# Shinokawa/Fast-SCNN-pytorch

Measured on AMD Instinct MI355X. Metric: images/sec fwd+bwd @1024x2048 bs=8 per GPU; 1/2/4/8-GPU scaling, higher is better.
Workload: dtype bf16; 1 GPU; cfg3 train step: fwd + CE(ignore -1) + bwd + fused SGD (fused low-res upsample+CE head); model=FastSCNN (19 classes), global_batch=8, per_gpu_batch=8, parallelism=dp1

## Files before the change

fast-scnn-pytorch_amd/_lib.py:

```python
import ctypes
import os
import threading

_HERE = os.path.dirname(os.path.abspath(__file__))
LIB_PATH = os.environ.get("FSCNN_LIB", os.path.join(_HERE, "libfastscnn_hip.so"))

DT_F32, DT_BF16, DT_F16 = 0, 1, 2
DT_U8 = 3

c_int, c_ll, c_float, c_vp, c_char_p = (ctypes.c_int, ctypes.c_longlong, ctypes.c_float,
                                        ctypes.c_void_p, ctypes.c_char_p)
c_ull, c_double = ctypes.c_ulonglong, ctypes.c_double
P_int, P_ll, P_vp = ctypes.POINTER(c_int), ctypes.POINTER(c_ll), ctypes.POINTER(c_vp)
P_float = ctypes.POINTER(c_float)
P_double = ctypes.POINTER(c_double)

SIGNATURES = {
    "fscnn_version": (c_char_p, []),
    "fscnn_last_error": (c_char_p, []),
    "fscnn_net_create": (c_int, [c_int, c_int, P_vp]),
    "fscnn_net_destroy": (None, [c_vp]),
    "fscnn_net_param_count": (c_int, [c_vp, P_int, P_ll]),
    "fscnn_net_param_info": (c_int, [c_vp, c_int, ctypes.POINTER(c_char_p), P_ll, P_ll]),
    "fscnn_net_buffer_count": (c_int, [c_vp, P_int, P_ll, P_int]),
# ... 58 lines not shown
    "fscnn_dice_head_ws_bytes": (c_ll, [c_vp]),
    "fscnn_forward_loss_dice": (c_int, [c_vp, c_vp, c_int, c_vp, c_float, c_float, c_float,
                                        c_float, c_float, c_vp, c_vp, c_vp, c_vp, c_vp, c_vp, c_vp,
                                        c_ull, c_float, c_float, c_vp]),
    "fscnn_backward_loss_dice": (c_int, [c_vp, c_vp, c_vp, c_float, c_float, c_float, c_vp, c_int,
                                         c_vp, c_vp, c_vp, c_vp, c_vp, c_ull, c_float, c_int,
                                         c_int, c_vp]),
    "fscnn_forward_loss_ohem": (c_int, [c_vp, c_vp, c_int, c_vp, c_ll, c_float, c_ll, c_vp, c_vp,
                                        c_vp, c_vp, c_vp, c_vp, c_vp, c_vp, c_vp, c_vp, c_ull,
                                        c_float, c_float, c_vp]),
    "fscnn_backward_dx": (c_int, [c_vp, c_vp, c_vp, c_vp, c_vp, c_vp, c_int, c_vp, c_int, c_vp,
                                  c_vp, c_vp, c_vp, c_ull, c_float, c_int, c_int, c_vp]),
    "fscnn_prof_begin": (c_int, [c_int, c_int]),
    "fscnn_prof_end": (c_int, [ctypes.POINTER(ctypes.c_double), P_ll, ctypes.POINTER(ctypes.c_double),
                               ctypes.POINTER(ctypes.c_double)]),
    "fscnn_prof_launch": (c_int, [c_ll, ctypes.POINTER(c_int), ctypes.POINTER(ctypes.c_float),
                                  ctypes.POINTER(ctypes.c_double), ctypes.POINTER(ctypes.c_double),
                                  ctypes.POINTER(c_char_p)]),
    "fscnn_prof_kind_name": (c_char_p, [c_int]),
    "fscnn_ce_parts": (c_ll, [c_int, c_ll]),
    "fscnn_ce_fwd": (c_int, [c_vp, c_int, c_vp, c_int, c_int, c_ll, c_ll, c_vp, c_vp, c_vp]),
    "fscnn_ce_bwd": (c_int, [c_vp, c_int, c_vp, c_int, c_int, c_ll, c_ll, c_vp, c_vp, c_vp,
                             c_vp]),
    "fscnn_sgd": (c_int, [c_vp, c_vp, c_vp, c_ll, c_float, c_float, c_float, c_float, c_int,
                          c_int, c_float, c_vp]),
    "fscnn_adamw": (c_int, [c_vp, c_vp, c_vp, c_vp, c_vp, c_ll, c_double, c_double, c_double,
                            c_double, c_double, c_int, c_int, c_vp, c_int, c_vp, c_vp, c_vp]),
    "fscnn_adamw_segments": (c_int, [c_vp, c_vp, c_vp, c_vp, c_vp, c_vp, c_vp, c_int, c_vp, c_int,
                                     c_vp, c_int, c_vp, c_int, c_int, c_vp, c_vp, c_vp]),
    "fscnn_conv0_fwd": (c_int, [c_vp, c_int, c_int, c_int, c_int, c_vp, c_vp, c_vp, c_int, c_vp,
                                c_int, c_vp]),
    "fscnn_conv0_wgrad_slab_floats": (c_ll, [c_int, c_int, c_int]),
    "fscnn_conv0_wgrad": (c_int, [c_vp, c_int, c_int, c_int, c_int, c_vp, c_int, c_vp, c_vp, c_vp]),
    "fscnn_dw3x3_fwd": (c_int, [c_vp, c_int, c_int, c_int, c_int, c_int, c_int, c_vp, c_vp, c_vp,
                                c_int, c_vp, c_vp]),
    "fscnn_dw3x3_dgrad": (c_int, [c_vp, c_int, c_int, c_int, c_int, c_int, c_int, c_vp, c_vp,
                                  c_vp]),
    "fscnn_dw3x3_wgrad_slab_floats": (c_ll, [c_int, c_int, c_int, c_int, c_int, c_int]),
    "fscnn_dw3x3_wgrad": (c_int, [c_vp, c_vp, c_int, c_int, c_int, c_int, c_int, c_int, c_vp,
                                  c_vp, c_vp]),
    "fscnn_pw_gemm": (c_int, [c_int, c_int, c_int, c_vp, c_int, c_vp, c_int, c_int, c_vp, c_vp,
                              c_vp, c_int, c_int, c_vp, c_int, c_vp, c_int, c_vp]),
    "fscnn_pw_dgrad_bnbwd": (c_int, [c_int, c_int, c_int, c_vp, c_int, c_vp, c_int, c_vp, c_int,
                                     c_vp, c_int, c_vp, c_int, c_vp, c_vp, c_vp, c_vp, c_int,
                                     c_vp, c_vp, c_vp, c_vp, c_vp, c_vp, c_int, P_int, c_vp]),
    "fscnn_kth_smallest": (c_int, [c_vp, c_ll, c_ll, c_vp, c_vp, c_vp]),
    "fscnn_debug_stamps": (c_int, [c_vp, c_int]),
    "fscnn_debug_stamp_count": (c_int, []),
    "fscnn_debug_stamp_tag": (c_char_p, [c_int]),
    "fscnn_pw_wgrad_slab_floats": (c_ll, [c_int, c_int, c_int]),
    "fscnn_pw_gemm_stats_parts": (c_int, [c_int, c_int, c_int, c_int, c_int, c_int]),
    "fscnn_pw_wgrad": (c_int, [c_int, c_int, c_int, c_vp, c_int, c_vp, c_int, c_vp, c_vp, c_int,
                               c_vp]),
    "fscnn_bn_finalize": (c_int, [c_vp, c_int, c_int, c_vp, c_vp, c_vp, c_vp, c_vp, c_float,
                                  c_vp, c_vp, c_vp, c_vp, c_vp]),
    "fscnn_bilinear_ac_fwd": (c_int, [c_vp, c_int, c_int, c_int, c_int, c_int, c_int, c_int,
                                      c_vp, c_int, c_int, c_vp]),
    "fscnn_bilinear_ac_bwd": (c_int, [c_vp, c_int, c_int, c_int, c_int, c_int, c_int, c_int,
                                      c_vp, c_vp, c_vp]),
    "fscnn_pyramid_pool_fwd": (c_int, [c_vp, c_int, c_int, c_int, c_int, c_int, c_int, c_vp,
                                       c_vp]),
    "fscnn_block_ir_fwd": (c_int, [c_vp, c_int, c_int, c_int, c_int, c_int, c_int, c_int, c_int,
                                   c_vp, c_vp, c_vp, c_vp, c_vp, c_vp, c_vp, c_vp, c_vp, c_int,
                                   c_vp, c_int, c_vp]),
    "fscnn_pyramid_pool_bwd": (c_int, [c_vp, c_int, c_int, c_int, c_int, c_int, c_vp, c_int,
                                       c_int, c_vp]),
    "fscnn_block_ir_s2_fwd": (c_int, [c_vp, c_int, c_int, c_int, c_int, c_int, c_int, c_int, c_int,
                                      c_vp, c_vp, c_vp, c_vp, c_vp, c_vp, c_vp, c_vp, c_vp, c_vp,
                                      c_int, c_vp]),
    "fscnn_block_ltd_fwd": (c_int, [c_vp, c_int, c_int, c_int, c_int, c_int, c_vp, c_vp, c_vp,
                                    c_vp, c_vp, c_vp, c_vp, c_vp, c_vp, c_vp, c_int, c_vp]),
    "fscnn_block_dsconv_fwd": (c_int, [c_vp, c_int, c_int, c_int, c_int, c_int, c_int, c_vp, c_vp,
                                       c_vp, c_vp, c_vp, c_vp, c_vp, c_int, c_vp]),
    "fscnn_block_dsconv_res_fwd": (c_int, [c_vp, c_int, c_int, c_int, c_int, c_int, c_int, c_int,
                                           c_int, c_vp, c_vp, c_vp, c_vp, c_vp, c_vp, c_vp, c_int,
                                           c_vp, c_int, c_vp]),
    "fscnn_block_cls_fwd": (c_int, [c_vp, c_int, c_int, c_int, c_int] + [c_vp] * 14 + [c_int, c_vp, c_vp,
                                                                              c_int, c_vp]),
    "fscnn_block_ffm_fwd": (c_int, [c_vp, c_int, c_int, c_int, c_int, c_int, c_int, c_vp, c_int,
                                    c_vp, c_vp, c_vp, c_vp, c_vp, c_vp, c_vp, c_vp, c_vp, c_vp,
                                    c_int, c_vp]),
}

_lib = None
_lock = threading.Lock()


def load():
    global _lib
    if _lib is not None:
        return _lib
    with _lock:
        if _lib is not None:
            return _lib
        if not os.path.exists(LIB_PATH):
            raise RuntimeError(
                "libfastscnn_hip.so not found at %s — build it with "
                "`python -c 'import __graft_entry__; __graft_entry__.build()'` "
                "(there is no CPU fallback)" % LIB_PATH)
        import torch
        lib = ctypes.CDLL(LIB_PATH, mode=ctypes.RTLD_GLOBAL)
        for name, (res, args) in SIGNATURES.items():
            fn = getattr(lib, name)
            fn.restype = res
            fn.argtypes = args
        _lib = lib
# ... 34 lines not shown
```

fast-scnn-pytorch_amd/csrc/capi.cpp:

```cpp
#include <algorithm>
#include <chrono>
#include <cmath>
#include <cstdlib>
#include <cstdarg>
#include <cstdio>
#include <cstring>
#include <new>
#include <string>

#include "../../include/fastscnn.h"
#include "net.hpp"

namespace fscnn {

static thread_local char g_err[512] = "";

void set_error(const char* fmt, ...) {
  va_list ap;
  va_start(ap, fmt);
  vsnprintf(g_err, sizeof g_err, fmt, ap);
  va_end(ap);
}
const char* last_error() { return g_err; }

// ... 961 lines not shown

int fscnn_pw_gemm_stats_parts(int M, int N, int K, int lda, int ldc, int dtype) {
  GemmArgs a{};
  static float dummy;
  a.M = M; a.N = N; a.K = K; a.lda = lda; a.ldb = K; a.ldc = ldc; a.part = &dummy;
  return gemm_nt_parts(a, dtype);
}
int fscnn_pw_gemm(int M, int N, int K, const void* A, int lda, const void* B, int ldb,
                  int b_trans, const float* scale, const float* shift, const void* R, int ldr,
                  int relu, void* C, int ldc, float* stats_part, int dtype, void* stream) {
  GemmArgs a{};
  a.M = M; a.N = N; a.K = K; a.A = A; a.lda = lda; a.B = B; a.ldb = ldb; a.b_trans = b_trans;
  a.scale = scale; a.shift = shift; a.R = R; a.ldr = ldr; a.relu = relu; a.C = C; a.ldc = ldc;
  a.part = stats_part;
  return gemm_nt(a, dtype, S(stream));
}
int fscnn_pw_dgrad_bnbwd(int M, int N, int K, const void* D, int ldd, const void* B, int ldb,
                         const void* R, int ldr, void* dX, int lddx, const void* z, int ldz,
                         const float* mean, const float* invstd, const float* scale,
                         const float* shift, int relu_mode, float* part, unsigned* counters,
                         double* tsum, float* dgamma, float* dbeta, float* coef, int dtype,
                         int* path, void* stream) {
  if (!D || !B || !dX || !z || !mean || !invstd || !scale || !shift || !part || !counters ||
      !tsum || !dgamma || !dbeta || !coef) {
    set_error("fscnn_pw_dgrad_bnbwd: null argument");
    return E_INVALID;
  }
  if (dtype < DT_F32 || dtype > DT_F16 || (relu_mode != 0 && relu_mode != 2)) {
    set_error("fscnn_pw_dgrad_bnbwd: dtype %d / relu_mode %d", dtype, relu_mode);
    return E_INVALID;
  }
  GemmArgs a{};
  a.M = M; a.N = N; a.K = K; a.A = D; a.lda = ldd; a.B = B; a.ldb = ldb; a.b_trans = 0;
  a.R = R; a.ldr = ldr; a.C = dX; a.ldc = lddx;
  a.bpart = part; a.bz = z; a.ldbz = ldz;
  a.bmean = mean; a.binvstd = invstd; a.bscale = scale; a.bshift = shift; a.bmode = relu_mode;
  a.tail.counters = counters; a.tail.tsum = tsum; a.tail.count = (double)M;
  a.tail.dgamma = dgamma; a.tail.dbeta = dbeta; a.tail.coef = coef;
  if (path) *path = gemm_stream_ok(a, dtype) ? 1 : 0;
  return gemm_nt(a, dtype, S(stream));
}
long long fscnn_pw_wgrad_slab_floats(int M, int N, int K) {
  return (long long)gemm_tn_splits(M, N, K) * N * K;
}
int fscnn_pw_wgrad(int M, int N, int K, const void* D, int ldd, const void* X, int ldx,
                   float* slab, float* dW, int dtype, void* stream) {
  GemmTnArgs a{};
  a.M = M; a.N = N; a.K = K; a.D = D; a.ldd = ldd; a.X = X; a.ldx = ldx; a.slab = slab;
  int s = gemm_tn_splits(M, N, K);
  int rc = gemm_tn(a, s, dtype, S(stream));
  if (rc) return rc;
  return reduce_slabs(slab, s, (long long)N * K, (long long)N * K, dW, 0, S(stream));
}

int fscnn_bn_finalize(float* part, int P, int C, const float* gamma, const float* beta,
                      float* rmean, float* rvar, long long* nbt, float momentum, float* mean,
                      float* invstd, float* scale, float* shift, void* stream) {
  BnFinalizeArgs a{};
  a.part = part; a.P = P; a.C = C; a.gamma = gamma; a.beta = beta; a.rmean = rmean;
  a.rvar = rvar; a.nbt = nbt; a.momentum = momentum; a.mean = mean; a.invstd = invstd;
  a.scale = scale; a.shift = shift;
  return bn_finalize(a, S(stream));
}

int fscnn_bilinear_ac_fwd(const void* x, int dtype, int N, int Hi, int Wi, int C, int Ho, int Wo,
                          void* y, int out_nchw, int out_dtype, void* stream) {
  UpArgs a{};
  a.N = N; a.Hi = Hi; a.Wi = Wi; a.C = C; a.Ho = Ho; a.Wo = Wo; a.x = x; a.ldx = C; a.y = y;
  a.ldy = C;
  if (out_nchw) return up_nchw(a, dtype, out_dtype, S(stream));
  return up_nhwc(a, dtype, S(stream));
}
int fscnn_bilinear_ac_bwd(const void* dy, int dtype, int N, int Hi, int Wi, int C, int Ho, int Wo,
                          float* tmp, void* dx, void* stream) {
  AxisBwdArgs a{};
  a.n_o1 = (long long)N * Ho; a.n_o2 = 1; a.Lout = Wo; a.Lin = Wi; a.n_in = C;
  a.g = dy; a.g_s1 = (long long)Wo * C; a.g_idx = C; a.g_in = 1;
  a.d = tmp; a.d_s1 = (long long)Wi * C; a.d_idx = C; a.d_in = 1;
  int rc = axis_bwd(a, dtype, DT_F32, S(stream));
  if (rc) return rc;
  AxisBwdArgs b{};
  b.n_o1 = N; b.n_o2 = 1; b.Lout = Ho; b.Lin = Hi; b.n_in = (long long)Wi * C;
  b.g = tmp; b.g_s1 = (long long)Ho * Wi * C; b.g_idx = (long long)Wi * C; b.g_in = 1;
  b.d = dx; b.d_s1 = (long long)Hi * Wi * C; b.d_idx = (long long)Wi * C; b.d_in = 1;
  return axis_bwd(b, DT_F32, dtype, S(stream));
}
int fscnn_pyramid_pool_fwd(const void* x, int dtype, int N, int H, int W, int C, int ldx,
                           void* pooled, void* stream) {
  PoolArgs a{};
  a.N = N; a.H = H; a.W = W; a.C = C; a.x = x; a.ldx = ldx; a.pooled = pooled;
  return pyramid_pool(a, dtype, S(stream));
}
int fscnn_pyramid_pool_bwd(const void* dpooled, int dtype, int N, int H, int W, int C, void* dx,
                           int lddx, int accumulate, void* stream) {
  PoolBwdArgs a{};
  a.N = N; a.H = H; a.W = W; a.C = C; a.dpooled = dpooled; a.dx = dx; a.lddx = lddx;
  a.accumulate = accumulate;
  return pyramid_pool_bwd(a, dtype, S(stream));
}

int fscnn_block_ir_fwd(const void* x, int ldx, int dtype, int N, int H, int W, int cin, int expand,
                       int cout, const void* w_expand, const float* w_dw, const void* w_project,
                       const float* scale_e, const float* shift_e, const float* scale_d,
                       const float* shift_d, const float* scale_p, const float* shift_p,
                       int residual, void* y, int ldy, void* stream) {
  if (!x || !y || !w_expand || !w_dw || !w_project || !scale_e || !shift_e || !scale_d ||
// ... 190 lines not shown
```

fast-scnn-pytorch_amd/csrc/gemm.hip:

```cpp
#include "bn_finish.hpp"

namespace fscnn {


constexpr int G_BM = 128;
constexpr int G_VROW = 8;
constexpr int G_VPAD = 9;
constexpr int G_ATMAX = 768;

template <typename T>
struct MfmaOp;

template <>
struct MfmaOp<float> {
  static __device__ __forceinline__ void run(const uint4& a, const uint4& b, f32x4& acc) {
    acc = __builtin_amdgcn_mfma_f32_16x16x4f32(__uint_as_float(a.x), __uint_as_float(b.x), acc, 0, 0, 0);
    acc = __builtin_amdgcn_mfma_f32_16x16x4f32(__uint_as_float(a.y), __uint_as_float(b.y), acc, 0, 0, 0);
    acc = __builtin_amdgcn_mfma_f32_16x16x4f32(__uint_as_float(a.z), __uint_as_float(b.z), acc, 0, 0, 0);
    acc = __builtin_amdgcn_mfma_f32_16x16x4f32(__uint_as_float(a.w), __uint_as_float(b.w), acc, 0, 0, 0);
  }
};

template <>
struct MfmaOp<bf16> {
  static __device__ __forceinline__ void run(const uint4& a, const uint4& b, f32x4& acc) {
    i16x8 av, bv;
    __builtin_memcpy(&av, &a, 16);
    __builtin_memcpy(&bv, &b, 16);
    acc = __builtin_amdgcn_mfma_f32_16x16x32_bf16(av, bv, acc, 0, 0, 0);
  }
};

template <>
struct MfmaOp<f16> {
  static __device__ __forceinline__ void run(const uint4& a, const uint4& b, f32x4& acc) {
    h16x8 av, bv;
    __builtin_memcpy(&av, &a, 16);
    __builtin_memcpy(&bv, &b, 16);
    acc = __builtin_amdgcn_mfma_f32_16x16x32_f16(av, bv, acc, 0, 0, 0);
  }
};

template <typename T>
__device__ __forceinline__ uint4 zero_tail(uint4 v, int valid) {
  constexpr int V = VecW<T>::V;
  uint32_t w[4] = {v.x, v.y, v.z, v.w};
  if (V == 4) {
#pragma unroll
    for (int j = 0; j < 4; ++j) w[j] = j < valid ? w[j] : 0u;
  } else {
#pragma unroll
    for (int j = 0; j < 4; ++j) {
// ... 650 lines not shown
  };
  using Pair = typename std::conditional<sizeof(T) == 2, uint32_t, uint2>::type;
  if (mb < me) load(mb);
  for (int mc = mb; mc < me; mc += TN_MC) {
    mask(mc);
    __syncthreads();
#pragma unroll
    for (int i = 0; i < PAIRS; ++i) {
      const int id = tid + 256 * i;
      const int rp = id / VPR, vv = id - rp * VPR;
      const T* d0 = reinterpret_cast<const T*>(&rd[i][0]);
      const T* d1 = reinterpret_cast<const T*>(&rd[i][1]);
      const T* x0 = reinterpret_cast<const T*>(&rx[i][0]);
      const T* x1 = reinterpret_cast<const T*>(&rx[i][1]);
#pragma unroll
      for (int j = 0; j < V; ++j) {
        const int n = vv * V + j;
        const int off = n * LD + swz(n, 2 * rp);
        Pair pd, px;
        __builtin_memcpy(reinterpret_cast<T*>(&pd), d0 + j, sizeof(T));
        __builtin_memcpy(reinterpret_cast<T*>(&pd) + 1, d1 + j, sizeof(T));
        __builtin_memcpy(reinterpret_cast<T*>(&px), x0 + j, sizeof(T));
        __builtin_memcpy(reinterpret_cast<T*>(&px) + 1, x1 + j, sizeof(T));
        *reinterpret_cast<Pair*>(&sDt[off]) = pd;
        *reinterpret_cast<Pair*>(&sXt[off]) = px;
      }
    }
    __syncthreads();
    if (mc + TN_MC < me) load(mc + TN_MC);
#pragma unroll
    for (int ks = 0; ks < TN_MC / 32; ++ks) {
      const int kb = ks * 32 + 8 * lq;
#pragma unroll
      for (int i = 0; i < 2; ++i)
#pragma unroll
        for (int j = 0; j < 2; ++j) {
          const int na = wn + i * 16 + li, nb = wk + j * 16 + li;
          TnOps<T>::mma(&sDt[na * LD + swz(na, kb)], &sXt[nb * LD + swz(nb, kb)], acc[i][j]);
        }
    }
  }
  float* sl = a.slab + (size_t)split * a.N * a.K;
#pragma unroll
  for (int i = 0; i < 2; ++i)
#pragma unroll
    for (int j = 0; j < 2; ++j)
#pragma unroll
      for (int r = 0; r < 4; ++r) {
        int n = n0 + wn + i * 16 + lq * 4 + r, k = k0 + wk + j * 16 + li;
        if (n < a.N && k < a.K) sl[(size_t)n * a.K + k] = acc[i][j][r];
      }
}

int gemm_tn_splits(int M, int N, int K) {
  constexpr int target = 512;
  int tiles = cdiv(N, TN_T) * cdiv(K, TN_T);
  int s = target / tiles;
  int smax = cdiv(M, 4 * TN_MC);
  if (s > smax) s = smax;
  if (s >= 8) s &= ~7;
  if (s < 1) s = 1;
  return s;
}

int gemm_tn(GemmTnArgs a, int splits, int dtype, hipStream_t st) {
  const int V = dtype == DT_F32 ? 4 : 8;
  if (a.ldd % V || a.ldx % V || (uintptr_t)a.D % 16 || (uintptr_t)a.X % 16) {
    set_error("gemm_tn: operands must be 16-B aligned (ldd=%d ldx=%d)", a.ldd, a.ldx);
    return E_INVALID;
  }
  a.rows_per_split = cdiv(cdiv(a.M, splits), TN_MC) * TN_MC;
  a.splits = splits;
  dim3 grid(cdiv(a.N, TN_T) * cdiv(a.K, TN_T) * splits);
  const double E = dtype == DT_F32 ? 4.0 : 2.0;
  const double M = a.M, N = a.N, K = a.K;
  ProfScope ps(PK_GEMM_TN, st, E * (M * N + M * K) + 4.0 * N * K, 2.0 * M * N * K);
  const bool xt = a.x_scale != nullptr;
  if (xt && (!a.x_shift || a.K % V)) {
    set_error("gemm_tn: lazy BN on X needs x_shift and K %% %d == 0", V);
    return E_UNSUPPORTED;
  }
#define TN_LAUNCH(T)                                        \
  do {                                                      \
    if (xt) prof_launch(gemm_tn_kernel<T, true>, grid, 256, 0, st, a); \
    else prof_launch(gemm_tn_kernel<T, false>, grid, 256, 0, st, a);   \
  } while (0)
  if (dtype == DT_F32) TN_LAUNCH(float);
  else if (dtype == DT_F16) TN_LAUNCH(f16);
  else TN_LAUNCH(bf16);
#undef TN_LAUNCH
  return check_launch("gemm_tn");
}

constexpr int RED_Q = 64;

__global__ void reduce_fold_kernel(float* slab, int S, int Q, long long stride, int count) {
  int i = blockIdx.x * blockDim.x + threadIdx.x;
  int q = blockIdx.y;
  if (i >= count) return;
  float s = 0.f;
  for (int k0 = q; k0 < S; k0 += 8 * Q) {
    float v[8];
#pragma unroll
    for (int u = 0; u < 8; ++u) {
      const int k = k0 + u * Q;
      const float t = slab[(size_t)(k < S ? k : q) * stride + i];
      v[u] = k < S ? t : 0.f;
    }
#pragma unroll
    for (int u = 0; u < 8; ++u) s += v[u];
  }
  slab[(size_t)q * stride + i] = s;
}

__global__ void reduce_final_kernel(const float* slab, int S, long long stride, int count,
                                    float* out, int accumulate, int C9) {
  int i = blockIdx.x * blockDim.x + threadIdx.x;
  if (i >= count) return;
  float s = 0.f;
  for (int k0 = 0; k0 < S; k0 += 8) {
    float v[8];
#pragma unroll
    for (int u = 0; u < 8; ++u) {
      const float t = slab[(size_t)(k0 + u < S ? k0 + u : 0) * stride + i];
      v[u] = k0 + u < S ? t : 0.f;
    }
#pragma unroll
    for (int u = 0; u < 8; ++u) s += v[u];
  }
  int o = C9 ? (i % C9) * 9 + i / C9 : i;
  out[o] = accumulate ? out[o] + s : s;
}

int reduce_slabs_ex(float* slab, int S, long long stride, long long count, float* out,
                    int accumulate, int C9, hipStream_t st) {
  if (count <= 0 || count > 0x7fffffff) { set_error("reduce_slabs: bad count"); return E_INVALID; }
  int n = (int)count;
  int S2 = S;
  if (S > RED_Q) {
    dim3 g1(cdiv(n, 256), RED_Q);
    prof_launch(reduce_fold_kernel, g1, 256, 0, st, slab, S, RED_Q, stride, n);
    S2 = RED_Q;
// ... 125 lines not shown
```

fast-scnn-pytorch_amd/csrc/kernels.hpp:

```cpp
#pragma once
#include "common.hpp"

namespace fscnn {

constexpr int MAX_FOLD = 48;
constexpr double BN_FROZEN_COUNT = -1.0;


struct Conv0Args {
  const void* x;
  int x_bf16;
  int N, H, W, Ho, Wo;
  const float* w;
  const float* scale;
  const float* shift;
  int relu;
  void* y;
  float* part;
  unsigned long long* stamps = nullptr;
};

struct Conv0WgradArgs {
  const void* x;
  int x_bf16;
// ... 459 lines not shown
  unsigned long long* stamps = nullptr;
};
bool ds2_ok(const Ds2Args& a);
int ds2_fwd(const Ds2Args& a, int dtype, hipStream_t st);
int ds_rows(int N, int H, int W);
int ds_fwd(const DsArgs& a, int dtype, hipStream_t st);

struct Conv0DgradArgs {
  const void* dz;
  const float* w;
  int N, H, W, Ho, Wo;
  void* dx;
  int dx_dtype;
};
int conv0_dgrad(const Conv0DgradArgs& a, int dz_dtype, hipStream_t st);
int conv0_parts(int N, int Ho, int Wo);
int conv0_fwd(const Conv0Args& a, int y_dtype, hipStream_t st);
int conv0_wgrad_parts(int N, int Ho, int Wo, int rows_per_block);
int conv0_wgrad(const Conv0WgradArgs& a, int dz_dtype, hipStream_t st);

constexpr int LC0_SLAB = 2 * 864 + 27;
struct LtdC0BwdArgs {
  int N, H, W;
  int Ho, Wo;
  const void* dy;
  const float* w;
  BnBwdPart bs{};
  BnTail tail{};
  const void* x;
  int x_dtype, XH, XW;
  float* slab;
};
int ltd_c0_bwd_parts(int N, int H, int W);
bool ltd_c0_bwd_ok(int dtype, int x_dtype, int XW, const void* x);
int ltd_c0_bwd(const LtdC0BwdArgs& a, int dtype, hipStream_t st);
int conv0_wgrad_combine(const float* sums, const float* tab, const float* mean, float* dw,
                        hipStream_t st);

int dw_parts(int N, int Ho, int Wo, int C, int dtype, int stride);
int dw_fwd(const DwArgs& a, int dtype, hipStream_t st);
int dw_dgrad(const DwBwdArgs& a, int dtype, hipStream_t st);
int dw_dgrad_parts(int N, int H, int W, int C, int dtype, int stride);
int dw_wgrad_parts(int N, int Ho, int Wo, int C, int dtype, int stride);
int dw_wgrad(const DwBwdArgs& a, int dtype, hipStream_t st);
int dw_wgrad_reduce(float* slab, int P, int C, float* dw, hipStream_t st);

int gemm_parts(int M);
int gemm_nt(const GemmArgs& a, int dtype, hipStream_t st);
bool gemm_stream_ok(const GemmArgs& a, int dtype);
int gemm_stream(const GemmArgs& a, int dtype, hipStream_t st);
int gemm_stream_parts(const GemmArgs& a, int dtype);
int gemm_nt_parts(const GemmArgs& a, int dtype);
int gemm_tn_splits(int M, int N, int K);
int gemm_tn(GemmTnArgs a, int splits, int dtype, hipStream_t st);
int reduce_slabs(float* slab, int S, long long stride, long long count, float* out,
                 int accumulate, hipStream_t st);
int reduce_slabs_ex(float* slab, int S, long long stride, long long count, float* out,
                    int accumulate, int C9, hipStream_t st);
constexpr int RED_MAXJOBS = 64;
struct RedJob {
  float* slab;
  float* out;
  long long stride;
  int S, count, accumulate, C9;
  int Q = 0;
};
struct RedTable {
  int n = 0;
  int blocks = 0;
  int blk0[RED_MAXJOBS + 1] = {};
  RedJob j[RED_MAXJOBS];
};
int reduce_slabs_multi(const RedTable& t, hipStream_t st);
int colsum_parts(int M);
int colsum(const void* D, int M, int N, int ld, float* part, int dtype, hipStream_t st);

int bn_fold(const FoldTable& t, hipStream_t st);
int bn_finalize(const BnFinalizeArgs& a, hipStream_t st);
int bn_apply(const BnApplyArgs& a, int dtype, hipStream_t st);
int bn_bwd_parts(long long M, int C, int dtype, int* rows_per_block);
int bn_bwd_reduce(const BnBwdArgs& a, int dtype, hipStream_t st);
int bn_bwd_finalize(float* part, int P, int C, double count, float* dgamma, float* dbeta,
                    float* coef, hipStream_t st, unsigned* counters = nullptr,
                    const BnBwdTab& tab = BnBwdTab());
int bn_bwd_apply(const BnBwdArgs& a, int dtype, hipStream_t st);

int up_nhwc(const UpArgs& a, int dtype, hipStream_t st);
int up_nchw(const UpArgs& a, int in_dtype, int out_dtype, hipStream_t st);
bool up_nchw_rows_path(const UpArgs& a);
int up_argmax(const UpArgs& a, int in_dtype, void* labels, int label_u8, hipStream_t st);
int seg_metric(const void* pred, int pred_u8, const long long* target, long long n, int C,
               long long* counts, hipStream_t st);
int axis_bwd(const AxisBwdArgs& a, int g_dtype, int d_dtype, hipStream_t st);
int pyramid_pool(const PoolArgs& a, int dtype, hipStream_t st);
int pyramid_pool_bwd(const PoolBwdArgs& a, int dtype, hipStream_t st);
int ppm_up_fwd(const PpmUpArgs& a, int dtype, hipStream_t st);
int ppm_up_bwd(const PpmUpArgs& a, void* dfeats, int dtype, hipStream_t st);

bool ppm_branches_ok(int maxM, int K, int dtype);
int ppm_branches_fwd(const PpmFwdArgs& a, int dtype, hipStream_t st);
int ppm_branches_bwd(const PpmBwdArgs& a, int dtype, hipStream_t st);

int ce_parts(int N, long long HW);
int ce_fwd(const CeArgs& a, float* out, int dtype, hipStream_t st);
int ce_bwd(const CeArgs& a, const float* gout, const float* stats, int dtype, hipStream_t st);
int ohem_prob(const CeArgs& a, float thresh, float* prob, unsigned long long* counts, int dtype,
              hipStream_t st);
// ... 100 lines not shown
```

fast-scnn-pytorch_amd/csrc/net.cpp:

```cpp
#include "net.hpp"
#include "bn_finish.hpp"

#include <cstdlib>
#include <cstring>
#include <functional>
#include <mutex>
#include <vector>

#include <cstdio>
#include <cstring>

namespace fscnn {

namespace {
struct Builder {
  Net& n;
  explicit Builder(Net& net) : n(net) {}
  long long palloc(const std::string& name, std::vector<int> shape) {
    long long numel = 1;
    for (int s : shape) numel *= s;
    long long off = (n.p_total + 15) / 16 * 16;
    n.params.push_back({name, shape, off, numel});
    n.p_total = off + numel;
    return off;
// ... 284 lines not shown
    pl.named.push_back({u.key + ".shift", u.shift, 1, u.C, u.C, 0});
    pl.named.push_back({u.key + ".mean", u.mean, 1, u.C, u.C, 0});
    pl.named.push_back({u.key + ".invstd", u.invstd, 1, u.C, u.C, 0});
  });
  nm("concat", pl.concat, M5, 256, 256, 0);
  nm("up_low", pl.up_low, M2, 128, 128, 0);
  nm("f", pl.f, M2, 128, 128, 0);
  nm("drop", pl.drop, M2, 128, 128, 0);
  nm("logits", pl.logits, M2, net.num_classes, pl.Cp, 0);

  if (train) {
    const int C = net.num_classes;
    pl.g_logits = B.get((size_t)M2 * pl.Cp * E);
    pl.t_up = B.get((size_t)N * C * H * pl.W3 * 4);
    pl.g_drop = B.get((size_t)M2 * 128 * E);
    gunit(pl.c2pw);
    gunit(pl.c2dw);
    gunit(pl.c1pw);
    gunit(pl.c1dw);
    pl.g_f = B.get((size_t)M2 * 128 * E);
    gunit(pl.fdw);
    pl.g_up = B.get((size_t)M2 * 128 * E);
    pl.t_up2 = B.get((size_t)N * pl.H3 * pl.W5 * 128 * 4);
    gunit(pl.po);
    pl.g_concat = B.get((size_t)M5 * 256 * E);
    pl.g_feats = B.get((size_t)50 * N * 32 * E);
    for (int i = 0; i < 4; ++i)
      gunit(pl.ppk[i], pl.g_feats + (size_t)PPM_BASE[i] * N * 32 * E, 32);
    pl.g_pooled = B.get((size_t)50 * N * 128 * E);
    for (int i = 8; i >= 0; --i) {
      gunit(pl.lbd[i]);
      gunit(pl.lbe[i]);
      gunit(pl.lbp[i], i == 8 ? pl.g_concat : OWN, i == 8 ? 256 : 0);
    }
    gunit(pl.l2pw);
    gunit(pl.l2dw);
    gunit(pl.l1pw);
    gunit(pl.l1dw);
    gunit(pl.c0);
    if (net.aux) {
      gunit(pl.aux0);
      pl.g_auxlog = B.get((size_t)M2 * pl.Cp * E);
      pl.g_aux = B.get((size_t)M2 * 32 * E);
      pl.aux_dcol = B.get((size_t)M2 * 576 * E);
    }
    size_t dzs = 0;
    for_each_unit(pl, [&](const Unit& u) { dzs += ((size_t)u.M * u.C * E + 255) / 256 * 256; });
    pl.dz_bytes = dzs;
    pl.dz = B.get(dzs);
    size_t slab = 0;
    auto add_slab = [&](size_t floats) { slab += (floats + 63) / 64 * 64; };
    auto pw_slab = [&](const ConvL& c, long long M) {
      const int k = c.cin * c.k * c.k;
      add_slab((size_t)gemm_tn_splits((int)M, c.cout, k) * c.cout * k);
      if (c.b >= 0) add_slab((size_t)colsum_parts((int)M) * c.cout);
    };
    for_each_unit(pl, [&](const Unit& u) {
      if (u.kind == U_PW) pw_slab(*u.conv, u.M);
      if (u.kind == U_DW)
        add_slab((size_t)dw_wgrad_parts(N, u.Ho, u.Wo, u.C, dtype, u.stride) * 9 * u.C);
    });
    pw_slab(net.cls_out, M2);
    if (net.aux) pw_slab(net.aux4, M2);
    add_slab((size_t)conv0_wgrad_parts(N, pl.H1, pl.W1, 8) * 864);
    add_slab((size_t)ltd_c0_bwd_parts(N, pl.H1, pl.W1) * LC0_SLAB);
    pl.slab_floats = slab;
    pl.slab = B.get(slab * 4);
    size_t bnp = 0;
    auto bnp_max = [&](size_t s) { if (s > bnp) bnp = s; };
    for_each_unit(pl, [&](const Unit& u) {
      int rpb;
      bnp_max((size_t)bn_bwd_parts(u.M, u.C, dtype, &rpb) * 2 * u.C);
      bnp_max((size_t)gemm_parts((int)u.M) * 2 * u.C);
      if (u.kind == U_DW)
        bnp_max((size_t)dw_dgrad_parts(N, u.Hi, u.Wi, u.C, dtype, u.stride) * 2 * u.C);
    });
    {
      int rpb;
      bnp_max((size_t)2 * bn_bwd_parts(pl.flow.M, 128, dtype, &rpb) * 2 * 128);
    }
    pl.bnpart = B.get(bnp * 4);
    pl.bnpart_floats = bnp;
    pl.coef = B.get(2 * 1024 * 4);
    pl.xtab = B.get((size_t)pl.c0.C * BWDX_STRIDE * 4);
    pl.c0sum = B.get((size_t)LC0_SLAB * 4);
    pl.cspart = B.get((size_t)colsum_parts((int)M2) * (C > 128 ? C : 128) * 4);
    pl.bws_bytes = B.top;
    for_each_unit(pl, [&](const Unit& u) {
      const bool ppk = &u >= pl.ppk && &u < pl.ppk + 4;
      if (u.ga_ld && !ppk && &u != &pl.aux0)
        pl.named.push_back({u.key + ".ga", u.ga, u.M, u.C, u.ga_ld, 1});
    });
    nm("g_logits", pl.g_logits, M2, C, pl.Cp, 1);
    nm("g_f", pl.g_f, M2, 128, 128, 1);
    nm("g_up", pl.g_up, M2, 128, 128, 1);
    nm("g_concat", pl.g_concat, M5, 256, 256, 1);
    nm("dz", pl.dz, M0, 32, 32, 1);
  }
  return OK;
}

struct SideStream {
  hipStream_t s = nullptr;
  hipEvent_t fork = nullptr, join = nullptr;
  int dev = -1;
  bool ready = false, failed = false;
  std::mutex mu;
// ... 1448 lines not shown
```

include/fastscnn.h:

```cpp
#ifndef FASTSCNN_H
#define FASTSCNN_H

#ifdef __cplusplus
extern "C" {
#endif

typedef struct fscnn_net fscnn_net;
typedef struct fscnn_plan fscnn_plan;

const char* fscnn_version(void);
const char* fscnn_last_error(void);

int fscnn_net_create(int num_classes, int aux, fscnn_net** out);
void fscnn_net_destroy(fscnn_net* net);
int fscnn_net_param_count(const fscnn_net* net, int* count, long long* total_floats);
int fscnn_net_param_info(const fscnn_net* net, int i, const char** name, long long* offset,
                         long long* numel);
int fscnn_net_buffer_count(const fscnn_net* net, int* count, long long* total_floats, int* num_bn);
int fscnn_net_buffer_info(const fscnn_net* net, int i, const char** name, long long* offset,
                          long long* numel);
int fscnn_net_stage_range(const fscnn_net* net, int stage, long long* begin, long long* end);

int fscnn_plan_create(const fscnn_net* net, int N, int H, int W, int dtype, int train,
                      fscnn_plan** out);
// ... 202 lines not shown
              float dampening, float weight_decay, int nesterov, int first, float grad_scale,
              void* stream);

int fscnn_adamw(float* p, const float* g, float* exp_avg, float* exp_avg_sq,
                float* max_exp_avg_sq, long long n, double lr, double beta1, double beta2,
                double eps, double weight_decay, int amsgrad, int maximize, float* step, int tick,
                const float* grad_scale, const float* found_inf, void* stream);
#define FSCNN_ADAMW_CHUNK 2048
#define FSCNN_ADAMW_MAX_GROUPS 8
typedef struct fscnn_adamw_seg {
  long long begin, end;
  int group;
  int chunk0;
} fscnn_adamw_seg;
typedef struct fscnn_adamw_group {
  double lr, beta1, beta2, eps, weight_decay;
  int amsgrad, maximize;
  int step_slot;
} fscnn_adamw_group;
int fscnn_adamw_segments(float* p, const float* g, float* exp_avg, float* exp_avg_sq,
                         float* max_exp_avg_sq, const fscnn_adamw_seg* segs,
                         const fscnn_adamw_seg* host_segs, int nseg, const int* chunk_seg,
                         int nchunks, const fscnn_adamw_group* groups, int ngroups, float* steps,
                         int nslots, int tick, const float* grad_scale, const float* found_inf,
                         void* stream);

int fscnn_conv0_fwd(const void* x, int x_dtype, int N, int H, int W, const float* w,
                    const float* scale, const float* shift, int relu, void* y, int y_dtype,
                    void* stream);
long long fscnn_conv0_wgrad_slab_floats(int N, int H, int W);
int fscnn_conv0_wgrad(const void* x, int x_dtype, int N, int H, int W, const void* dz,
                      int dz_dtype, float* slab, float* dw, void* stream);
int fscnn_dw3x3_fwd(const void* x, int dtype, int N, int H, int W, int C, int stride,
                    const float* w, const float* scale, const float* shift, int relu, void* y,
                    void* stream);
int fscnn_dw3x3_dgrad(const void* dy, int dtype, int N, int H, int W, int C, int stride,
                      const float* w, void* dx, void* stream);
long long fscnn_dw3x3_wgrad_slab_floats(int N, int H, int W, int C, int stride, int dtype);
int fscnn_dw3x3_wgrad(const void* x, const void* dy, int dtype, int N, int H, int W, int C,
                      int stride, float* slab, float* dw, void* stream);
int fscnn_pw_gemm_stats_parts(int M, int N, int K, int lda, int ldc, int dtype);
int fscnn_pw_gemm(int M, int N, int K, const void* A, int lda, const void* B, int ldb,
                  int b_trans, const float* scale, const float* shift, const void* R, int ldr,
                  int relu, void* C, int ldc, float* stats_part, int dtype, void* stream);
int fscnn_pw_dgrad_bnbwd(int M, int N, int K, const void* D, int ldd, const void* B, int ldb,
                         const void* R, int ldr, void* dX, int lddx, const void* z, int ldz,
                         const float* mean, const float* invstd, const float* scale,
                         const float* shift, int relu_mode, float* part, unsigned* counters,
                         double* tsum, float* dgamma, float* dbeta, float* coef, int dtype,
                         int* path, void* stream);
long long fscnn_pw_wgrad_slab_floats(int M, int N, int K);
int fscnn_pw_wgrad(int M, int N, int K, const void* D, int ldd, const void* X, int ldx,
                   float* slab, float* dW, int dtype, void* stream);
int fscnn_bn_finalize(float* part, int P, int C, const float* gamma, const float* beta,
                      float* rmean, float* rvar, long long* nbt, float momentum, float* mean,
                      float* invstd, float* scale, float* shift, void* stream);
int fscnn_bilinear_ac_fwd(const void* x, int dtype, int N, int Hi, int Wi, int C, int Ho, int Wo,
                          void* y, int out_nchw, int out_dtype, void* stream);
int fscnn_bilinear_ac_bwd(const void* dy, int dtype, int N, int Hi, int Wi, int C, int Ho, int Wo,
                          float* tmp, void* dx, void* stream);
int fscnn_pyramid_pool_fwd(const void* x, int dtype, int N, int H, int W, int C, int ldx,
                           void* pooled, void* stream);
int fscnn_pyramid_pool_bwd(const void* dpooled, int dtype, int N, int H, int W, int C, void* dx,
                           int lddx, int accumulate, void* stream);

#ifdef __cplusplus
}
#endif
#endif
```

Baseline: 1463 images/s.

## Add transposed-LDS-read wgrad GEMM kernel and lower default split target

Adds a new TN weight-gradient GEMM kernel that stages D and X chunks in swizzled shared memory and feeds 16x16x32 bf16/f16 MFMAs through ds_read_tr16_b64 transposed reads, with a three-deep register prefetch ring. This kernel is enabled only through the FSCNN_TN_TR environment flag or an explicit variant argument, plus new C API entry points for testing. Separately, the default split-K target for the wgrad GEMM drops from 512 to 384 tiles, while slab allocation still sizes for 512 so buffers stay large enough. With default settings only the split-count change takes effect, trading fewer partial slabs to reduce for less parallelism per GEMM.

```diff
diff --git a/fast-scnn-pytorch_amd/_lib.py b/fast-scnn-pytorch_amd/_lib.py
--- a/fast-scnn-pytorch_amd/_lib.py
+++ b/fast-scnn-pytorch_amd/_lib.py
@@ -134,6 +134,10 @@
     "fscnn_pw_gemm_stats_parts": (c_int, [c_int, c_int, c_int, c_int, c_int, c_int]),
     "fscnn_pw_wgrad": (c_int, [c_int, c_int, c_int, c_vp, c_int, c_vp, c_int, c_vp, c_vp, c_int,
                                c_vp]),
+    "fscnn_pw_wgrad_ex_slab_floats": (c_ll, [c_int, c_int, c_int, c_int]),
+    "fscnn_pw_wgrad_ex": (c_int, [c_int, c_int, c_int, c_vp, c_int, c_vp, c_int, c_vp, c_vp, c_int,
+                                  c_int, c_vp, c_vp, c_int, c_vp]),
+    "fscnn_tn_tr_launches": (c_ll, []),
     "fscnn_bn_finalize": (c_int, [c_vp, c_int, c_int, c_vp, c_vp, c_vp, c_vp, c_vp, c_float,
                                   c_vp, c_vp, c_vp, c_vp, c_vp]),
     "fscnn_bilinear_ac_fwd": (c_int, [c_vp, c_int, c_int, c_int, c_int, c_int, c_int, c_int,
diff --git a/fast-scnn-pytorch_amd/csrc/capi.cpp b/fast-scnn-pytorch_amd/csrc/capi.cpp
--- a/fast-scnn-pytorch_amd/csrc/capi.cpp
+++ b/fast-scnn-pytorch_amd/csrc/capi.cpp
@@ -1037,6 +1037,25 @@
   if (rc) return rc;
   return reduce_slabs(slab, s, (long long)N * K, (long long)N * K, dW, 0, S(stream));
 }
+long long fscnn_pw_wgrad_ex_slab_floats(int M, int N, int K, int splits) {
+  return (long long)(splits > 0 ? splits : gemm_tn_splits(M, N, K)) * N * K;
+}
+int fscnn_pw_wgrad_ex(int M, int N, int K, const void* D, int ldd, const void* X, int ldx,
+                      const float* x_scale, const float* x_shift, int splits, int variant,
+                      float* slab, float* dW, int dtype, void* stream) {
+  if (M < 1 || N < 1 || K < 1 || dtype < DT_F32 || dtype > DT_F16 || variant < 0 || variant > 1) {
+    set_error("fscnn_pw_wgrad_ex: M %d N %d K %d dtype %d variant %d", M, N, K, dtype, variant);
+    return E_INVALID;
+  }
+  GemmTnArgs a{};
+  a.M = M; a.N = N; a.K = K; a.D = D; a.ldd = ldd; a.X = X; a.ldx = ldx; a.slab = slab;
+  a.x_scale = x_scale; a.x_shift = x_shift;
+  const int s = splits > 0 ? splits : gemm_tn_splits(M, N, K);
+  int rc = gemm_tn(a, s, dtype, S(stream), variant);
+  if (rc || !dW) return rc;
+  return reduce_slabs(slab, s, (long long)N * K, (long long)N * K, dW, 0, S(stream));
+}
+long long fscnn_tn_tr_launches(void) { return gemm_tn_tr_launches(); }
 
 int fscnn_bn_finalize(float* part, int P, int C, const float* gamma, const float* beta,
                       float* rmean, float* rvar, long long* nbt, float momentum, float* mean,
diff --git a/fast-scnn-pytorch_amd/csrc/gemm.hip b/fast-scnn-pytorch_amd/csrc/gemm.hip
--- a/fast-scnn-pytorch_amd/csrc/gemm.hip
+++ b/fast-scnn-pytorch_amd/csrc/gemm.hip
@@ -1,3 +1,5 @@
+#include <atomic>
+
 #include "bn_finish.hpp"
 
 namespace fscnn {
@@ -754,8 +756,157 @@
       }
 }
 
-int gemm_tn_splits(int M, int N, int K) {
-  constexpr int target = 512;
+constexpr int TR_RING = 3;
+
+__device__ __forceinline__ i16x4 tn_tr(const unsigned char* p) {
+  return __builtin_amdgcn_ds_read_tr16_b64_v4i16((__attribute__((address_space(3))) i16x4*)p);
+}
+template <typename T>
+__device__ __forceinline__ void tn_tr_mma(const i16x4& a0, const i16x4& a1, const i16x4& b0,
+                                          const i16x4& b1, f32x4& acc) {
+  const i16x8 av = __builtin_shufflevector(a0, a1, 0, 1, 2, 3, 4, 5, 6, 7);
+  const i16x8 bv = __builtin_shufflevector(b0, b1, 0, 1, 2, 3, 4, 5, 6, 7);
+  if constexpr (std::is_same<T, f16>::value) {
+    h16x8 ah, bh;
+    __builtin_memcpy(&ah, &av, 16);
+    __builtin_memcpy(&bh, &bv, 16);
+    acc = __builtin_amdgcn_mfma_f32_16x16x32_f16(ah, bh, acc, 0, 0, 0);
+  } else {
+    acc = __builtin_amdgcn_mfma_f32_16x16x32_bf16(av, bv, acc, 0, 0, 0);
+  }
+}
+
+template <typename T, bool XT>
+__global__ __launch_bounds__(256) void gemm_tn_kernel_tr(GemmTnArgs a) {
+  static_assert(sizeof(T) == 2, "ds_read_b64_tr_b16 is 16-bit only");
+  constexpr int V = 8;
+  constexpr int ROWB = TN_T * 2;
+  constexpr int IMG = TN_MC * ROWB;
+  __shared__ __attribute__((aligned(16))) unsigned char s_raw[2 * 2 * IMG];
+  const int tid = threadIdx.x, lane = tid & 63, wave = tid >> 6;
+  const int li = lane & 15, lq = lane >> 4;
+  const int tiles_k = cdiv(a.K, TN_T);
+  int split, tile;
+  xcd_tile(blockIdx.x, a.splits, cdiv(a.N, TN_T) * tiles_k, split, tile);
+  const int tn = tile / tiles_k, tk = tile - tn * tiles_k;
+  const int n0 = tn * TN_T, k0 = tk * TN_T;
+  const int wn = (wave >> 1) * 32, wk = (wave & 1) * 32;
+  const int mb = split * a.rows_per_split;
+  const int me = min(a.M, mb + a.rows_per_split);
+  const int nch = mb < me ? cdiv(me - mb, TN_MC) : 0;
+  const T* D = (const T*)a.D;
+  const T* X = (const T*)a.X;
+
+  f32x4 acc[2][2];
+#pragma unroll
+  for (int i = 0; i < 2; ++i)
+#pragma unroll
+    for (int j = 0; j < 2; ++j) acc[i][j] = f32x4{0.f, 0.f, 0.f, 0.f};
+
+  const int rp = tid >> 3, vv = tid & 7;
+  const int n = n0 + vv * V, k = k0 + vv * V;
+  const int wo = ROWB * rp + 16 * (vv ^ (2 * (((rp >> 1) & 1) | (((rp >> 3) & 1) << 1))));
+  const size_t od = (size_t)(mb + rp) * a.ldd + n, ox = (size_t)(mb + rp) * a.ldx + k;
+  auto load = [&](uint4 (&d)[2], uint4 (&x)[2], int c) {
+#pragma unroll
+    for (int h = 0; h < 2; ++h) {
+      const int r = c * TN_MC + 32 * h;
+      const bool okm = mb + r + rp < me;
+      const size_t pd = od + (size_t)r * a.ldd, px = ox + (size_t)r * a.ldx;
+      d[h] = *reinterpret_cast<const uint4*>(D + (okm && n < a.N ? pd : 0));
+      x[h] = *reinterpret_cast<const uint4*>(X + (okm && k < a.K ? px : 0));
+    }
+  };
+  float xsc[XT ? V : 1], xsh[XT ? V : 1];
+  if constexpr (XT) {
+#pragma unroll
+    for (int j = 0; j < V; ++j) {
+      const int kk = k + j < a.K ? k + j : 0;
+      xsc[j] = a.x_scale[kk];
+      xsh[j] = a.x_shift[kk];
+    }
+  }
+  auto stage = [&](const uint4 (&d)[2], const uint4 (&x)[2], int c, unsigned char* buf) {
+#pragma unroll
+    for (int h = 0; h < 2; ++h) {
+      const bool okm = mb + c * TN_MC + rp + 32 * h < me;
+      uint4 xv = x[h];
+      if constexpr (XT) xv = bnrelu_vec<T>(xv, xsc, xsh);
+      *reinterpret_cast<uint4*>(buf + wo + 32 * ROWB * h) = zero_tail<T>(d[h], okm ? a.N - n : 0);
+      *reinterpret_cast<uint4*>(buf + IMG + wo + 32 * ROWB * h) = zero_tail<T>(xv, okm ? a.K - k : 0);
+    }
+  };
+  int ao[2], bo[2];
+  {
+    const int q = li >> 2, p = li & 3;
+    const int row = 8 * lq + q;
+    const int f = 2 * (((q >> 1) & 1) | ((lq & 1) << 1));
+#pragma unroll
+    for (int i = 0; i < 2; ++i) {
+      ao[i] = ROWB * row + 16 * ((((wn >> 3) + 2 * i + (p >> 1)) ^ f)) + 8 * (p & 1);
+      bo[i] = IMG + ROWB * row + 16 * ((((wk >> 3) + 2 * i + (p >> 1)) ^ f)) + 8 * (p & 1);
+    }
+  }
+  auto mult = [&](const unsigned char* buf) {
+#pragma unroll
+    for (int ks = 0; ks < TN_MC / 32; ++ks) {
+      i16x4 fa[2][2], fb[2][2];
+#pragma unroll
+      for (int i = 0; i < 2; ++i)
+#pragma unroll
+        for (int h = 0; h < 2; ++h) {
+          fa[i][h] = tn_tr(buf + ao[i] + ROWB * (32 * ks + 4 * h));
+          fb[i][h] = tn_tr(buf + bo[i] + ROWB * (32 * ks + 4 * h));
+        }
+#pragma unroll
+      for (int i = 0; i < 2; ++i)
+#pragma unroll
+        for (int j = 0; j < 2; ++j)
+          tn_tr_mma<T>(fa[i][0], fa[i][1], fb[j][0], fb[j][1], acc[i][j]);
+    }
+  };
+  auto step = [&](uint4 (&d)[2], uint4 (&x)[2], int c, bool refill) {
+    unsigned char* buf = s_raw + (c & 1) * (2 * IMG);
+    stage(d, x, c, buf);
+    if (refill) load(d, x, c + TR_RING);
+    __syncthreads();
+    mult(buf);
+  };
+  static_assert(TR_RING == 3, "the chunk loop is unrolled over three named register sets");
+  uint4 d0[2], x0[2], d1[2], x1[2], d2[2], x2[2];
+  int c = 0;
+  if (nch >= 2 * TR_RING) {
+    load(d0, x0, 0);
+    load(d1, x1, 1);
+    load(d2, x2, 2);
+    for (; c + 2 * TR_RING <= nch; c += TR_RING) {
+      step(d0, x0, c, true);
+      step(d1, x1, c + 1, true);
+      step(d2, x2, c + 2, true);
+    }
+  } else {
+    if (0 < nch) load(d0, x0, 0);
+    if (1 < nch) load(d1, x1, 1);
+    if (2 < nch) load(d2, x2, 2);
+  }
+  for (; c < nch; c += TR_RING) {
+    step(d0, x0, c, c + TR_RING < nch);
+    if (c + 1 < nch) step(d1, x1, c + 1, c + 1 + TR_RING < nch);
+    if (c + 2 < nch) step(d2, x2, c + 2, c + 2 + TR_RING < nch);
+  }
+  float* sl = a.slab + (size_t)split * a.N * a.K;
+#pragma unroll
+  for (int i = 0; i < 2; ++i)
+#pragma unroll
+    for (int j = 0; j < 2; ++j)
+#pragma unroll
+      for (int r = 0; r < 4; ++r) {
+        int nn = n0 + wn + i * 16 + lq * 4 + r, kk = k0 + wk + j * 16 + li;
+        if (nn < a.N && kk < a.K) sl[(size_t)nn * a.K + kk] = acc[i][j][r];
+      }
+}
+
+static int tn_splits_for(int target, int M, int N, int K) {
   int tiles = cdiv(N, TN_T) * cdiv(K, TN_T);
   int s = target / tiles;
   int smax = cdiv(M, 4 * TN_MC);
@@ -764,9 +915,23 @@
   if (s < 1) s = 1;
   return s;
 }
-
-int gemm_tn(GemmTnArgs a, int splits, int dtype, hipStream_t st) {
+int gemm_tn_splits(int M, int N, int K) { return tn_splits_for(384, M, N, K); }
+int gemm_tn_slab_splits(int M, int N, int K) { return tn_splits_for(512, M, N, K); }
+
+static bool tn_tr_on() {
+  static const bool on = env_on("FSCNN_TN_TR");
+  return on;
+}
+static std::atomic<long long> g_tn_tr_launches{0};
+long long gemm_tn_tr_launches() { return g_tn_tr_launches.load(); }
+
+int gemm_tn(GemmTnArgs a, int splits, int dtype, hipStream_t st, int variant) {
   const int V = dtype == DT_F32 ? 4 : 8;
+  if (variant > 0 && dtype == DT_F32) {
+    set_error("gemm_tn: the transposed-read kernel is 16-bit only");
+    return E_UNSUPPORTED;
+  }
+  const bool tr = dtype != DT_F32 && (variant < 0 ? tn_tr_on() : variant > 0);
   if (a.ldd % V || a.ldx % V || (uintptr_t)a.D % 16 || (uintptr_t)a.X % 16) {
     set_error("gemm_tn: operands must be 16-B aligned (ldd=%d ldx=%d)", a.ldd, a.ldx);
     return E_INVALID;
@@ -787,9 +952,19 @@
     if (xt) prof_launch(gemm_tn_kernel<T, true>, grid, 256, 0, st, a); \
     else prof_launch(gemm_tn_kernel<T, false>, grid, 256, 0, st, a);   \
   } while (0)
-  if (dtype == DT_F32) TN_LAUNCH(float);
+#define TN_LAUNCH_TR(T)                                        \
+  do {                                                         \
+    if (xt) prof_launch(gemm_tn_kernel_tr<T, true>, grid, 256, 0, st, a); \
+    else prof_launch(gemm_tn_kernel_tr<T, false>, grid, 256, 0, st, a);   \
+  } while (0)
+  if (tr) {
+    if (dtype == DT_F16) TN_LAUNCH_TR(f16);
+    else TN_LAUNCH_TR(bf16);
+    g_tn_tr_launches.fetch_add(1);
+  } else if (dtype == DT_F32) TN_LAUNCH(float);
   else if (dtype == DT_F16) TN_LAUNCH(f16);
   else TN_LAUNCH(bf16);
+#undef TN_LAUNCH_TR
 #undef TN_LAUNCH
   return check_launch("gemm_tn");
 }
diff --git a/fast-scnn-pytorch_amd/csrc/kernels.hpp b/fast-scnn-pytorch_amd/csrc/kernels.hpp
--- a/fast-scnn-pytorch_amd/csrc/kernels.hpp
+++ b/fast-scnn-pytorch_amd/csrc/kernels.hpp
@@ -535,7 +535,9 @@
 int gemm_stream_parts(const GemmArgs& a, int dtype);
 int gemm_nt_parts(const GemmArgs& a, int dtype);
 int gemm_tn_splits(int M, int N, int K);
-int gemm_tn(GemmTnArgs a, int splits, int dtype, hipStream_t st);
+int gemm_tn_slab_splits(int M, int N, int K);
+int gemm_tn(GemmTnArgs a, int splits, int dtype, hipStream_t st, int variant = -1);
+long long gemm_tn_tr_launches();
 int reduce_slabs(float* slab, int S, long long stride, long long count, float* out,
                  int accumulate, hipStream_t st);
 int reduce_slabs_ex(float* slab, int S, long long stride, long long count, float* out,
diff --git a/fast-scnn-pytorch_amd/csrc/net.cpp b/fast-scnn-pytorch_amd/csrc/net.cpp
--- a/fast-scnn-pytorch_amd/csrc/net.cpp
+++ b/fast-scnn-pytorch_amd/csrc/net.cpp
@@ -360,7 +360,7 @@
     auto add_slab = [&](size_t floats) { slab += (floats + 63) / 64 * 64; };
     auto pw_slab = [&](const ConvL& c, long long M) {
       const int k = c.cin * c.k * c.k;
-      add_slab((size_t)gemm_tn_splits((int)M, c.cout, k) * c.cout * k);
+      add_slab((size_t)gemm_tn_slab_splits((int)M, c.cout, k) * c.cout * k);
       if (c.b >= 0) add_slab((size_t)colsum_parts((int)M) * c.cout);
     };
     for_each_unit(pl, [&](const Unit& u) {
diff --git a/include/fastscnn.h b/include/fastscnn.h
--- a/include/fastscnn.h
+++ b/include/fastscnn.h
@@ -278,6 +278,11 @@
 long long fscnn_pw_wgrad_slab_floats(int M, int N, int K);
 int fscnn_pw_wgrad(int M, int N, int K, const void* D, int ldd, const void* X, int ldx,
                    float* slab, float* dW, int dtype, void* stream);
+long long fscnn_pw_wgrad_ex_slab_floats(int M, int N, int K, int splits);
+int fscnn_pw_wgrad_ex(int M, int N, int K, const void* D, int ldd, const void* X, int ldx,
+                      const float* x_scale, const float* x_shift, int splits, int variant,
+                      float* slab, float* dW, int dtype, void* stream);
+long long fscnn_tn_tr_launches(void);
 int fscnn_bn_finalize(float* part, int P, int C, const float* gamma, const float* beta,
                       float* rmean, float* rvar, long long* nbt, float momentum, float* mean,
                       float* invstd, float* scale, float* shift, void* stream);
```

Result: no change. 1477 images/s (median of 6 runs) (+1.0%).
